# eikehmueller/mlmcpathintegral

Measured on AMD Instinct MI355X. Metric: lattice-site-updates/sec, higher is better.
Workload: dtype f64

## Files before the change

mlmcpathintegral_amd/csrc/schwinger_sweeps.hip:

```cpp
#include <stdio.h>
#include <string.h>
#include <stdlib.h>

#include "lattice_sweep.hpp"
#include "schwinger_perm.hpp"
#include "step_envelope.hpp"
#include "vonmises.hpp"

namespace mlmcpi {

#ifdef MLMCPI_STAMPS
extern "C" int mlmcpi_debug_read_stamps(unsigned long long *h_out, uint32_t n_workgroups) {
  MLMCPI_HIP_TRY(hipDeviceSynchronize());
  MLMCPI_HIP_TRY(hipMemcpyFromSymbol(h_out, HIP_SYMBOL(g_stamps), (size_t)n_workgroups * 16 * sizeof(unsigned long long)));
  return MLMCPI_OK;
}
#endif

template <int NT, int S, bool DIRECT = false, class Setup, class Commit>
__device__ __forceinline__ void heatbath_region(uint32_t nr, uint32_t nc, const RngKey &key, HbPool &pool, Setup setup,
                                                Commit commit) {
  if (DIRECT) {
    heatbath_cells<NT, S>(nr * nc, key, pool,
                          [&](uint32_t idx, double &tau, double &centre, uint32_t &site, uint32_t &o) {
                            const uint32_t ri = idx / nc;
                            setup(ri, idx - ri * nc, tau, centre, site, o);
                          },
                          commit);
    return;
  }
  uint32_t cur = threadIdx.x, ri = cur / nc, ci = cur - ri * nc;
  const uint32_t dr = NT / nc, dc = NT - dr * nc;
  heatbath_cells<NT, S>(nr * nc, key, pool,
                        [&](uint32_t idx, double &tau, double &centre, uint32_t &site, uint32_t &o) {
                          while (cur < idx) {
                            cur += NT;
                            ri += dr;
                            ci += dc;
                            if (ci >= nc) {
                              ci -= nc;
                              ++ri;
                            }
                          }
                          setup(ri, ci, tau, centre, site, o);
                        },
                        commit);
}

template <int NT, int S, bool DIRECT, class E, class Setup, class KappaExact, class Commit>
__device__ __forceinline__ void heatbath_region_step(uint32_t nr, uint32_t nc, uint32_t origin, uint32_t row_stride,
                                                     uint32_t col_stride, const RngKey &key, VsPool<E> &pool, Setup setup,
                                                     KappaExact kappa_exact, Commit commit) {
  if (DIRECT) {
    heatbath_cells_step<NT, S, E>(nr * nc, key, pool,
                                  [&](uint32_t idx) {
                                    const uint32_t ri = idx / nc;
                                    return origin + ri * row_stride + (idx - ri * nc) * col_stride;
                                  },
                                  setup, kappa_exact, commit);
    return;
  }
  const float rcp = 1.0f / (float)nc;
  heatbath_cells_step<NT, S, E>(nr * nc, key, pool,
                                [&](uint32_t idx) {
                                  uint32_t ri = (uint32_t)(((float)idx + 0.5f) * rcp);
                                  int32_t ci = (int32_t)(idx - ri * nc);
                                  if (ci < 0) { --ri; ci += (int32_t)nc; }
                                  else if (ci >= (int32_t)nc) { ++ri; ci -= (int32_t)nc; }
                                  return origin + ri * row_stride + (uint32_t)ci * col_stride;
                                },
                                setup, kappa_exact, commit);
}

template <bool HEAT, int NT, int TWC = 0, int THC = 0, bool STEP = false>
__global__ void __launch_bounds__(NT, HEAT ? (NT == 256 ? 4 : NT == 512 ? 2 : 1) : 1)
    schwinger_sweep_kernel(uint32_t Mt, uint32_t Mx, double beta, const double2 *__restrict__ in,
                           double2 *__restrict__ out, TileGeom tg, uint32_t nsweeps_arg, uint32_t kinds, RngKey key0,
                           uint32_t pool_cap, int qoi_op, double *__restrict__ qoi_partial, const uint32_t *__restrict__ vs_table) {
  extern __shared__ double lds[];
  __shared__ double qoi_red[NT / kWave];
  constexpr bool FIXED = TWC > 0;
  const uint32_t nsweeps = FIXED ? 1u : nsweeps_arg;
  const uint32_t H = 2 * nsweeps;
  const uint32_t tile = blockIdx.x, b = blockIdx.y;
  const uint32_t ty = tile / tg.tiles_x, tx = tile - ty * tg.tiles_x;
  const uint32_t i0 = tx * (FIXED ? TWC : tg.TW), j0 = ty * (FIXED ? THC : tg.TH);
  const uint32_t ow = FIXED ? TWC : min(tg.TW, Mt - i0), oh = FIXED ? THC : min(tg.TH, Mx - j0);
  const uint32_t bw = ow + 2 * H, bh = oh + 2 * H;
  auto wrap = [&](uint32_t base, uint32_t off, uint32_t n) {
    if (FIXED) {
      const uint32_t v = base + off;
      return v >= n ? v - n : v;
    }
    return wrap_add(base, off, n);
  };
  using PoolEntry = typename std::conditional<FIXED, uint16_t, uint32_t>::type;
  double *pool_lds = lds;
  HbPool pool = HbPool::carve(pool_lds, HEAT && !STEP ? pool_cap : 0u);
  VsPool<PoolEntry> vpool = VsPool<PoolEntry>::carve(pool_lds, HEAT && STEP ? pool_cap : 0u, STEP ? vs_table : nullptr);
  double *th0 = lds + (HEAT ? sweep_pool_bytes(STEP, FIXED, pool_cap) / sizeof(double) : 0), *th1 = th0 + (size_t)bw * bh;
  const double beta2 = 2. * beta;
  const uint32_t sc = (uint32_t)(((uint64_t)i0 + Mt - (H % Mt)) % Mt);
  const uint32_t sr = (uint32_t)(((uint64_t)j0 + Mx - (H % Mx)) % Mx);
  const double2 *src = in + (size_t)b * Mt * Mx;
  RngKey key = key0;
  key.chain += b;

  stage_region<NT, (NT >= 1024 ? 3 : 5), double2>(
      bh, bw, [&](uint32_t r, uint32_t c) { return src[(size_t)wrap(sr, r, Mx) * Mt + wrap(sc, c, Mt)]; },
      [&](uint32_t r, uint32_t c, double2 v) {
        th0[r * bw + c] = v.x;
        th1[r * bw + c] = v.y;
      });
  __syncthreads();

  for (uint32_t s = 0; s < nsweeps; ++s) {
    const bool heat = HEAT && (FIXED || ((kinds >> s) & 1u));
    RngKey skey = key;
    skey.step += s;
    const bool last = s + 1 == nsweeps;
    const uint32_t r_hi0 = last ? H + oh : bh - 2;
    const uint32_t c_lo0 = last ? H - 1 : 0, c_hi0 = last ? H + ow : bw - 2;
    const uint32_t r_lo1 = last ? H : 0, r_hi1 = last ? H + oh - 1 : bh - 2;
    for (uint32_t par = 0; par < 2; ++par) {
      const uint32_t r_first = last ? H + par : (par ? 1 : 2);
      const uint32_t nr = r_first <= r_hi0 ? (r_hi0 - r_first) / 2 + 1 : 0;
      const uint32_t ncol = c_hi0 - c_lo0 + 1;
      if (heat && STEP) {
        heatbath_region_step<NT, 5, FIXED, PoolEntry>(
            nr, ncol, r_first * bw + c_lo0, 2 * bw, 1, skey, vpool,
            [&](uint32_t o, VsCell &cell) {
              const uint32_t r = o / bw, c = o - r * bw;
              vs_cell(beta2, th0[o + bw] + th1[o] - th1[o + 1], th0[o - bw] + th1[o - bw + 1] - th1[o - bw], cell);
              cell.site = 2 * (wrap(sr, r, Mx) * Mt + wrap(sc, c, Mt));
            },
            [&](uint32_t o) {
              return vs_kappa_exact(beta2, th0[o + bw] + th1[o] - th1[o + 1], th0[o - bw] + th1[o - bw + 1] - th1[o - bw]);
            },
            [&](uint32_t o, double v) { th0[o] = v; });
      } else if (heat) {
        heatbath_region<NT, 5, FIXED>(
            nr, ncol, skey, pool,
            [&](uint32_t ri, uint32_t ci, double &tau, double &centre, uint32_t &site, uint32_t &o) {
              const uint32_t r = r_first + 2 * ri, c = c_lo0 + ci;
              o = r * bw + c;
              const double tp = th0[o + bw] + th1[o] - th1[o + 1];
              const double tm = th0[o - bw] + th1[o - bw + 1] - th1[o - bw];
              expcos_params(beta, tp, tm, tau, centre);
              site = 2 * (wrap(sr, r, Mx) * Mt + wrap(sc, c, Mt));
            },
            [&](uint32_t o, double v) { th0[o] = v; });
      } else
      for_region<NT>(nr, ncol, [&](uint32_t ri, uint32_t ci) {
        const uint32_t r = r_first + 2 * ri, o = r * bw + c_lo0 + ci;
        const double tp = th0[o + bw] + th1[o] - th1[o + 1];
        const double tm = th0[o - bw] + th1[o - bw + 1] - th1[o - bw];
        th0[o] = mod_2pi_fast((tp + tm) - th0[o]);
      });
      __syncthreads();
    }
    for (uint32_t par = 0; par < 2; ++par) {
      const uint32_t c_first = last ? H + par : (par ? 1 : 2);
      const uint32_t c_hi1 = last ? (par ? H + ow - 1 : H + ow) : bw - 2;
      const uint32_t nc = c_first <= c_hi1 ? (c_hi1 - c_first) / 2 + 1 : 0;
      const uint32_t nrow = r_hi1 - r_lo1 + 1;
      if (heat && STEP) {
        heatbath_region_step<NT, 5, FIXED, PoolEntry>(
            nrow, nc, r_lo1 * bw + c_first, bw, 2, skey, vpool,
            [&](uint32_t o, VsCell &cell) {
              const uint32_t r = o / bw, c = o - r * bw;
              vs_cell(beta2, th0[o] + th1[o + 1] - th0[o + bw], th0[o + bw - 1] + th1[o - 1] - th0[o - 1], cell);
              cell.site = 2 * (wrap(sr, r, Mx) * Mt + wrap(sc, c, Mt)) + 1;
            },
            [&](uint32_t o) {
              return vs_kappa_exact(beta2, th0[o] + th1[o + 1] - th0[o + bw], th0[o + bw - 1] + th1[o - 1] - th0[o - 1]);
            },
            [&](uint32_t o, double v) { th1[o] = v; });
      } else if (heat) {
        heatbath_region<NT, 5, FIXED>(
            nrow, nc, skey, pool,
            [&](uint32_t ri, uint32_t ci, double &tau, double &centre, uint32_t &site, uint32_t &o) {
              const uint32_t r = r_lo1 + ri, c = c_first + 2 * ci;
              o = r * bw + c;
              const double tp = th0[o] + th1[o + 1] - th0[o + bw];
              const double tm = th0[o + bw - 1] + th1[o - 1] - th0[o - 1];
              expcos_params(beta, tp, tm, tau, centre);
              site = 2 * (wrap(sr, r, Mx) * Mt + wrap(sc, c, Mt)) + 1;
            },
            [&](uint32_t o, double v) { th1[o] = v; });
      } else
      for_region<NT>(nrow, nc, [&](uint32_t ri, uint32_t ci) {
        const uint32_t r = r_lo1 + ri, c = c_first + 2 * ci, o = r * bw + c;
        const double tp = th0[o] + th1[o + 1] - th0[o + bw];
        const double tm = th0[o + bw - 1] + th1[o - 1] - th0[o - 1];
        th1[o] = mod_2pi_fast((tp + tm) - th1[o]);
      });
      __syncthreads();
    }
  }

  double acc[1] = {0.0};
  double2 *dst = out + (size_t)b * Mt * Mx;
  for_region<NT>(oh, ow, [&](uint32_t r, uint32_t c) {
    const uint32_t o = (r + H) * bw + (c + H);
    dst[(size_t)(j0 + r) * Mt + (i0 + c)] = make_double2(th0[o], th1[o]);
    if (qoi_op) {
      const double thp = th0[o] + th1[o + 1] - th0[o + bw] - th1[o];
      acc[0] += qoi_op == 3 ? cos_reduced(thp) : mod_2pi(thp);
    }
  });
  if (qoi_op) {
    block_sum<1>(acc, qoi_red);
    if (threadIdx.x == 0) qoi_partial[(size_t)b * gridDim.x + blockIdx.x] = acc[0];
  }
}

template <int NT, bool STEP>
__device__ __forceinline__ void schwinger_image_heat(double *th0, double *th1, VsPool<uint32_t> &vpool, HbPool &hpool, uint32_t Mt,
                                                     uint32_t Mx, double beta, double2 *__restrict__ out, uint32_t i0, uint32_t j0,
                                                     uint32_t b, uint32_t tile, RngKey key0, int qoi_op,
                                                     double *__restrict__ qoi_partial, double *qoi_red) {
  constexpr int TW = 64, TH = 64, HB = 2, IW = TW + 2 * HB;
  constexpr uint32_t bw = IW;
  const uint32_t sc = i0 >= (uint32_t)HB ? i0 - HB : i0 + Mt - HB;
  const uint32_t sr = j0 >= (uint32_t)HB ? j0 - HB : j0 + Mx - HB;
  auto wrap = [](uint32_t base, uint32_t off, uint32_t n) {
    const uint32_t v = base + off;
    return v >= n ? v - n : v;
  };
  RngKey skey = key0;
  skey.chain += b;
  const double beta2 = 2. * beta;
  constexpr bool kMapped = STEP && 32 % (NT / kWave) == 0;
  constexpr uint32_t NW = NT / kWave, NIT = kMapped ? 32 / NW : 1;
  constexpr int kT1 = IW * (TH + 2 * HB) * 8;
  const uint32_t lds_th0 = (uint32_t)(uintptr_t)th0;
  const uint32_t wave = __builtin_amdgcn_readfirstlane(threadIdx.x / kWave), lane = threadIdx.x % kWave;
  for (uint32_t par = 0; par < 2; ++par) {
    const uint32_t r_first = HB + par, nr = (HB + TH - r_first) / 2 + 1;
    constexpr uint32_t ncol = TW + 2;
    if (!STEP)
      heatbath_region<NT, 5, true>(
          nr, ncol, skey, hpool,
          [&](uint32_t ri, uint32_t ci, double &tau, double &centre, uint32_t &site, uint32_t &o) {
            const uint32_t r = r_first + 2 * ri, c = HB - 1 + ci;
            o = r * bw + c;
            expcos_params(beta, th0[o + bw] + th1[o] - th1[o + 1], th0[o - bw] + th1[o - bw + 1] - th1[o - bw], tau, centre);
            site = 2 * (wrap(sr, r, Mx) * Mt + wrap(sc, c, Mt));
          },
          [&](uint32_t o, double v) { th0[o] = v; });
    else if constexpr (kMapped) {
      uint32_t o_next = (r_first + 2 * wave) * bw + (HB - 1) + lane;
      uint32_t srow = wrap(sr, r_first + 2 * wave, Mx);
      const uint32_t scol = wrap(sc, HB - 1 + lane, Mt), n_top = (nr - NIT * NW) * ncol;
      heatbath_cells_step_mapped<NT, NIT, uint32_t>(
          n_top + 2 * (NIT * NW), skey, vpool,
          [&](uint32_t &o, uint32_t &site) {
            o = o_next;
            site = (srow * Mt + scol) << 1;
            o_next += 2 * NW * bw;
            srow = wrap(srow, 2 * NW, Mx);
          },
          [&](uint32_t i) {
            const uint32_t j = i - n_top, ri = i < n_top ? (uint32_t)(NIT * NW) : j >> 1, ci = i < n_top ? i : 64 + (j & 1u);
            return (r_first + 2 * ri) * bw + (HB - 1) + ci;
          },
          [&](uint32_t o) {
            const uint32_t r = o / bw, c = o - r * bw;
            return 2 * (wrap(sr, r, Mx) * Mt + wrap(sc, c, Mt));
          },
          [&](uint32_t o, double (&v)[6]) {
            const uint32_t a = lds_th0 + (o - bw) * 8u;
            v[0] = lds_read_f64<2 * bw * 8>(a);
            v[1] = lds_read_f64<kT1 + bw * 8>(a);
            v[2] = lds_read_f64<kT1 + bw * 8 + 8>(a);
            v[3] = lds_read_f64<0>(a);
            v[4] = lds_read_f64<kT1 + 8>(a);
            v[5] = lds_read_f64<kT1>(a);
          },
          [&](const double (&v)[6], VsCell &cell) { vs_cell(beta2, v[0] + v[1] - v[2], v[3] + v[4] - v[5], cell); },
          [&](uint32_t o) {
            return vs_kappa_exact(beta2, th0[o + bw] + th1[o] - th1[o + 1], th0[o - bw] + th1[o - bw + 1] - th1[o - bw]);
          },
          [&](uint32_t o, double v) { th0[o] = v; });
    } else
    heatbath_region_step<NT, 5, true, uint32_t>(
        nr, ncol, r_first * bw + (HB - 1), 2 * bw, 1, skey, vpool,
        [&](uint32_t o, VsCell &cell) {
          const uint32_t r = o / bw, c = o - r * bw;
          vs_cell(beta2, th0[o + bw] + th1[o] - th1[o + 1], th0[o - bw] + th1[o - bw + 1] - th1[o - bw], cell);
          cell.site = 2 * (wrap(sr, r, Mx) * Mt + wrap(sc, c, Mt));
        },
        [&](uint32_t o) {
          return vs_kappa_exact(beta2, th0[o + bw] + th1[o] - th1[o + 1], th0[o - bw] + th1[o - bw + 1] - th1[o - bw]);
        },
        [&](uint32_t o, double v) { th0[o] = v; });
    __syncthreads();
    MLMCPI_STAMP(5 + par);
  }
  for (uint32_t par = 0; par < 2; ++par) {
    const uint32_t c_first = HB + par, c_hi1 = par ? HB + TW - 1 : HB + TW;
    const uint32_t nc = (c_hi1 - c_first) / 2 + 1;
    if (!STEP)
      heatbath_region<NT, 5, true>(
          TH, nc, skey, hpool,
          [&](uint32_t ri, uint32_t ci, double &tau, double &centre, uint32_t &site, uint32_t &o) {
            const uint32_t r = HB + ri, c = c_first + 2 * ci;
            o = r * bw + c;
            expcos_params(beta, th0[o] + th1[o + 1] - th0[o + bw], th0[o + bw - 1] + th1[o - 1] - th0[o - 1], tau, centre);
            site = 2 * (wrap(sr, r, Mx) * Mt + wrap(sc, c, Mt)) + 1;
          },
          [&](uint32_t o, double v) { th1[o] = v; });
    else if constexpr (kMapped) {
      const uint32_t r0 = HB + 2 * wave + (lane >> 5), c0 = c_first + 2 * (lane & 31u);
      uint32_t o_next = r0 * bw + c0;
      uint32_t rowmt = wrap(sr, r0, Mx) * Mt;
      const uint32_t scol = wrap(sc, c0, Mt), mxmt = Mx * Mt;
      heatbath_cells_step_mapped<NT, NIT, uint32_t>(
          (nc - 32) * (uint32_t)TH, skey, vpool,
          [&](uint32_t &o, uint32_t &site) {
            o = o_next;
            site = ((rowmt + scol) << 1) | 1u;
            o_next += 2 * NW * bw;
            rowmt += 2 * NW * Mt;
            rowmt = min(rowmt, rowmt - mxmt);
          },
          [&](uint32_t i) { return (HB + i) * bw + c_first + 64; },
          [&](uint32_t o) {
            const uint32_t r = o / bw, c = o - r * bw;
            return 2 * (wrap(sr, r, Mx) * Mt + wrap(sc, c, Mt)) + 1;
          },
          [&](uint32_t o, double (&v)[6]) {
            const uint32_t a = lds_th0 + (o - 1) * 8u;
            v[0] = lds_read_f64<8>(a);
            v[1] = lds_read_f64<kT1 + 16>(a);
            v[2] = lds_read_f64<bw * 8 + 8>(a);
            v[3] = lds_read_f64<bw * 8>(a);
            v[4] = lds_read_f64<kT1>(a);
            v[5] = lds_read_f64<0>(a);
          },
          [&](const double (&v)[6], VsCell &cell) { vs_cell(beta2, v[0] + v[1] - v[2], v[3] + v[4] - v[5], cell); },
          [&](uint32_t o) {
            return vs_kappa_exact(beta2, th0[o] + th1[o + 1] - th0[o + bw], th0[o + bw - 1] + th1[o - 1] - th0[o - 1]);
          },
          [&](uint32_t o, double v) { th1[o] = v; });
    } else
    heatbath_region_step<NT, 5, true, uint32_t>(
        TH, nc, HB * bw + c_first, bw, 2, skey, vpool,
        [&](uint32_t o, VsCell &cell) {
          const uint32_t r = o / bw, c = o - r * bw;
          vs_cell(beta2, th0[o] + th1[o + 1] - th0[o + bw], th0[o + bw - 1] + th1[o - 1] - th0[o - 1], cell);
          cell.site = 2 * (wrap(sr, r, Mx) * Mt + wrap(sc, c, Mt)) + 1;
        },
        [&](uint32_t o) {
          return vs_kappa_exact(beta2, th0[o] + th1[o + 1] - th0[o + bw], th0[o + bw - 1] + th1[o - 1] - th0[o - 1]);
        },
        [&](uint32_t o, double v) { th1[o] = v; });
    __syncthreads();
    MLMCPI_STAMP(7 + par);
  }

  double acc[1] = {0.0};
  double2 *dst = out + (size_t)b * Mt * Mx;
  for_region<NT>(TH, TW, [&](uint32_t r, uint32_t c) {
    if (j0 + r >= Mx || i0 + c >= Mt) return;
    const uint32_t o = (r + HB) * bw + (c + HB);
    store_streaming(&dst[(size_t)(j0 + r) * Mt + (i0 + c)], th0[o], th1[o]);
    if (qoi_op) {
      const double thp = th0[o] + th1[o + 1] - th0[o + bw] - th1[o];
      acc[0] += qoi_op == 3 ? cos_reduced(thp) : mod_2pi(thp);
    }
  });
  if (qoi_op) {
    block_sum<1>(acc, qoi_red);
    if (threadIdx.x == 0) qoi_partial[(size_t)b * gridDim.x + tile] = acc[0];
  }
  MLMCPI_STAMP(9);
}

template <int TH>
__global__ void __launch_bounds__(512, 4)
    schwinger_perm_kernel(uint32_t Mt, uint32_t Mx, const double2 *__restrict__ in, double2 *__restrict__ out, uint32_t tiles_x,
                          uint32_t K) {
  constexpr int NT = 512;
  using PG = PermGeom<NT, 0, TH>;
  extern __shared__ double lds[];
  const uint32_t tile = blockIdx.x, b = blockIdx.y;
  const uint32_t ty = tile / tiles_x, tx = tile - ty * tiles_x;
  const uint32_t i0 = tx * 64, j0 = ty * TH;
  double2 res[2][PG::NV];
  perm_sweeps<NT, 0, TH>(lds, in + (size_t)b * Mt * Mx, Mt, Mx, i0, j0, K, res);
  double *th0 = lds, *th1 = lds + 64 * TH;
  __syncthreads();
  perm_store_image<NT, 0, TH>(th0, th1, res);
  __syncthreads();
  double2 *dst = out + (size_t)b * Mt * Mx;
#pragma unroll
  for (int k = 0; k < 64 * TH / NT; ++k) {
    const uint32_t v = threadIdx.x + k * NT, r = v / 64, c = v % 64;
    if (j0 + r < Mx && i0 + c < Mt)
      store_streaming(&dst[(size_t)(j0 + r) * Mt + (i0 + c)], th0[v], th1[v]);
  }
}

template <int NT, bool STEP>
__global__ void __launch_bounds__(NT, 4)
    schwinger_perm_heat_kernel(uint32_t Mt, uint32_t Mx, double beta, const double2 *__restrict__ in, double2 *__restrict__ out,
                               uint32_t tiles_x, uint32_t K, RngKey key0, int qoi_op, double *__restrict__ qoi_partial,
                               const uint32_t *__restrict__ vs_table) {
  using PH = PermHeatGeom<NT, STEP>;
  using PG = typename PH::PG;
  using OH = typename PH::OH;
  constexpr int IW = OH::IW, IH = OH::IH;
  static_assert(PG::OW == IW && 2 * PG::HR == IH, "the closed-form stage fills the heat bath's image");
  extern __shared__ double lds[];
  __shared__ double qoi_red[NT / kWave];
  const uint32_t tile = blockIdx.x, b = blockIdx.y;
  const uint32_t ty = tile / tiles_x, tx = tile - ty * tiles_x;
  const uint32_t i0 = tx * 64, j0 = ty * 64;
  MLMCPI_STAMP(0);
  MLMCPI_STAMP_WHERE();
  uint32_t tabw = 0;
  if (STEP && threadIdx.x < kVsTableBytes / 4) tabw = vs_table[threadIdx.x];
  HbPool hpool = HbPool::carve(lds, STEP ? 0u : OH::hb_pool_cap);
  double *th0 = lds + OH::pool_bytes / sizeof(double), *th1 = th0 + IW * IH;
  double2 res[2][PG::NV];
  perm_sweeps<NT, 2>(th0, in + (size_t)b * Mt * Mx, Mt, Mx, i0, j0, K, res);
  MLMCPI_STAMP(3);
  VsPool<uint32_t> vpool = VsPool<uint32_t>::carve(lds, OH::pool_cap, nullptr);
  if (STEP) {
    if (threadIdx.x < kVsTableBytes / 4) reinterpret_cast<uint32_t *>(lds)[threadIdx.x] = tabw;
    if (threadIdx.x < 2) vpool.count[threadIdx.x] = 0;
    vpool.tab = VsTable::at(lds, vs_table);
  }
  __syncthreads();
  perm_store_image<NT, 2>(th0, th1, res);
  __syncthreads();
  MLMCPI_STAMP(4);
  schwinger_image_heat<NT, STEP>(th0, th1, vpool, hpool, Mt, Mx, beta, out, i0, j0, b, tile, key0, qoi_op, qoi_partial, qoi_red);
}

template <bool HEAT, int NT>
static int allow_full_lds() {
  MLMCPI_HIP_TRY(hipFuncSetAttribute((const void *)schwinger_sweep_kernel<HEAT, NT>, hipFuncAttributeMaxDynamicSharedMemorySize, 160 * 1024 - 256));
  if (HEAT)
    MLMCPI_HIP_TRY(hipFuncSetAttribute((const void *)schwinger_sweep_kernel<HEAT, NT, 0, 0, HEAT>, hipFuncAttributeMaxDynamicSharedMemorySize, 160 * 1024 - 256));
  return MLMCPI_OK;
}

int schwinger_allow_lds() {
  if (int rc = allow_full_lds<false, 256>()) return rc;
  if (int rc = allow_full_lds<true, 256>()) return rc;
  if (int rc = allow_full_lds<false, 512>()) return rc;
  if (int rc = allow_full_lds<true, 512>()) return rc;
  if (int rc = allow_full_lds<false, 1024>()) return rc;
  if (int rc = allow_full_lds<true, 1024>()) return rc;
  if (int rc = schwinger_or_block_allow_lds()) return rc;
  if (int rc = allow_lds((const void *)schwinger_perm_kernel<64>, kPermPlaneMax)) return rc;
  if (int rc = allow_lds((const void *)schwinger_perm_kernel<32>, kPermPlaneMax)) return rc;
  if (int rc = allow_lds((const void *)schwinger_perm_heat_kernel<512, true>, HeatImageGeom::hb_bytes)) return rc;
  if (int rc = allow_lds((const void *)schwinger_perm_heat_kernel<512, false>, HeatImageGeom::hb_bytes)) return rc;
  if (int rc = allow_lds((const void *)schwinger_perm_heat_kernel<1024, true>, 156 * 1024)) return rc;
  if (int rc = allow_lds((const void *)schwinger_perm_heat_kernel<1024, false>, 156 * 1024)) return rc;
  return MLMCPI_OK;
}

template <bool HEAT, int NT>
static void launch_tile_sweep_nt(const SweepLaunch &l, const SweepArgs &a) {
  const dim3 grid(l.grid_x, a.B);
  const TileGeom tg{l.tile_w, l.tile_h, l.tiles_x};
  const uint32_t n = l.n_overrelax + l.n_heatbath;
#define MLMCPI_SCHW_SWEEP(...)                                                                                                       \
  hipLaunchKernelGGL((schwinger_sweep_kernel<__VA_ARGS__>), grid, dim3(NT), l.lds_bytes, a.st, a.Mt, a.Mx, a.coupling, (const double2 *)a.src, \
                     (double2 *)a.dst, tg, n, l.kinds, a.key, l.pool_cap, a.qoi_op, a.qoi_partial, a.vs_table)
  if (l.fixed_tile && l.step) MLMCPI_SCHW_SWEEP(HEAT, NT, 64, 32, HEAT);
  else if (l.fixed_tile) MLMCPI_SCHW_SWEEP(HEAT, NT, 64, 32);
  else if (l.step) MLMCPI_SCHW_SWEEP(HEAT, NT, 0, 0, HEAT);
  else MLMCPI_SCHW_SWEEP(HEAT, NT);
#undef MLMCPI_SCHW_SWEEP
}

static int launch_tile_sweep(const SweepLaunch &l, const SweepArgs &a) {
  const bool heat = l.n_heatbath != 0;
  switch (l.threads) {
    case 1024: heat ? launch_tile_sweep_nt<true, 1024>(l, a) : launch_tile_sweep_nt<false, 1024>(l, a); break;
    case 512: heat ? launch_tile_sweep_nt<true, 512>(l, a) : launch_tile_sweep_nt<false, 512>(l, a); break;
    default: heat ? launch_tile_sweep_nt<true, 256>(l, a) : launch_tile_sweep_nt<false, 256>(l, a);
  }
  MLMCPI_LAUNCH_CHECK("lattice sweep kernel");
  return MLMCPI_OK;
}

static int launch_perm(const SweepLaunch &l, const SweepArgs &a) {
  const dim3 grid(l.grid_x, a.B);
  const double2 *in = (const double2 *)a.src;
  double2 *out = (double2 *)a.dst;
#define MLMCPI_PERM_HEAT(NT, STEP)                                                                                           \
  hipLaunchKernelGGL((schwinger_perm_heat_kernel<NT, STEP>), grid, dim3(NT), l.lds_bytes, a.st, a.Mt, a.Mx, a.coupling, in, out, \
                     l.tiles_x, l.n_overrelax, a.key, a.qoi_op, a.qoi_partial, a.vs_table)
  if (l.kernel == MLMCPI_K_SCHWINGER_PERM_HEAT) {
    if (l.threads == 1024 && l.step) MLMCPI_PERM_HEAT(1024, true);
    else if (l.threads == 1024) MLMCPI_PERM_HEAT(1024, false);
    else if (l.step) MLMCPI_PERM_HEAT(512, true);
    else MLMCPI_PERM_HEAT(512, false);
  } else if (l.tile_h == 64)
    hipLaunchKernelGGL(schwinger_perm_kernel<64>, grid, dim3(512), l.lds_bytes, a.st, a.Mt, a.Mx, in, out, l.tiles_x, l.n_overrelax);
  else
    hipLaunchKernelGGL(schwinger_perm_kernel<32>, grid, dim3(512), l.lds_bytes, a.st, a.Mt, a.Mx, in, out, l.tiles_x, l.n_overrelax);
#undef MLMCPI_PERM_HEAT
  MLMCPI_LAUNCH_CHECK("schwinger closed-form kernel");
  return MLMCPI_OK;
}

int schwinger_sweep_launch(const SweepLaunch &l, const SweepArgs &args) {
  SweepArgs a = args;
  if (l.n_heatbath) a.key.step += l.n_overrelax;
  void *partial = nullptr;
  if (l.step)
    if (int rc = vs_table_device(2. * a.coupling, &a.vs_table)) return rc;
  if (a.qoi_op)
    if (int rc = scratch((size_t)a.B * l.grid_x * sizeof(double), &partial, a.st)) return rc;
  a.qoi_partial = (double *)partial;
  int rc;
  switch (l.kernel) {
    case MLMCPI_K_SCHWINGER_PERM:
    case MLMCPI_K_SCHWINGER_PERM_HEAT: rc = launch_perm(l, a); break;
    case MLMCPI_K_SCHWINGER_OR_BLOCK: rc = schwinger_or_block_launch(l, a); break;
    default: rc = launch_tile_sweep(l, a);
  }
  if (!rc && a.qoi_op) rc = lattice_finish(a.qoi_partial, l.grid_x, a.B, a.qoi_op, 1.0 / ((double)a.Mx * a.Mt), a.d_qoi, a.d_acc, a.st);
  return rc;
}

int schwinger_site_updates(const mlmcpi_lattice_action *act, double *d_state, uint32_t B, const uint32_t *d_sites, uint32_t n,
                           uint32_t site, int32_t heat, uint64_t seed, uint32_t chain0, uint32_t step, hipStream_t st) {
  const uint32_t *vs_table = nullptr;
  if (heat && 2. * act->beta <= kVsKappaMax)
    if (int rc = vs_table_device(2. * act->beta, &vs_table)) return rc;
  hipLaunchKernelGGL((lattice_site_update_kernel<true>), dim3((B + 63) / 64), dim3(64), 0, st, act->Mt, act->Mx, act->beta, d_state, B,
                     d_sites, n, site, (int)heat, make_key(seed, chain0, step), vs_table);
  MLMCPI_LAUNCH_CHECK("lattice_site_update_kernel");
  return MLMCPI_OK;
}

}
```

mlmcpathintegral_amd/csrc/step_envelope.hpp:

```cpp
#pragma once
#include "device_common.hpp"
#include "vonmises.hpp"

namespace mlmcpi {

constexpr double kVsKappaMax = 16.0;
constexpr int kVsClasses = 8, kVsBins = 8, kVsSel = 64;
constexpr uint32_t kVsU2Bits = 22;
constexpr uint32_t kVsCodeOff = 0, kVsScrOff = 512, kVsLwOff = 576, kVsFinOff = 1088, kVsConstOff = 1216, kVsTableBytes = 1232;
__host__ __device__ constexpr uint32_t vs_edge16(uint32_t k) { return (0xC8643210u >> (4u * k)) & 15u; }
__host__ __device__ constexpr uint32_t vs_width16(uint32_t k) { return (0x44221111u >> (4u * k)) & 15u; }
constexpr float kVsU2Slack = 1100.0f;
__host__ __device__ inline float vs_band_of_scale(double scale) { return (float)(1e-5 * (1.0 + scale * 1.4426950408889634)); }

struct VsTable {
  const uint8_t *base;
  float s_acc, s_rej;
  __device__ static VsTable at(const void *image, const uint32_t *__restrict__ d_table) {
    VsTable t{(const uint8_t *)image, 0.f, 0.f};
    if (d_table) {
      t.s_acc = __uint_as_float(to_vgpr(d_table[kVsConstOff / 4]));
      t.s_rej = __uint_as_float(to_vgpr(d_table[kVsConstOff / 4 + 1]));
    }
    return t;
  }
  __device__ static VsTable stage(void *lds, const uint32_t *__restrict__ d_table) {
    if (d_table)
      for (uint32_t i = threadIdx.x; i < kVsTableBytes / 4; i += blockDim.x) ((uint32_t *)lds)[i] = d_table[i];
    return at(lds, d_table);
  }
  __device__ static VsTable in_global(const uint32_t *__restrict__ d_table) { return at(d_table, d_table); }
};

__device__ __forceinline__ float sinf_half_pi(float y) {
  const float y2 = y * y;
  float p = 2.600053086e-06f;
  p = fmaf(p, y2, -1.980661437e-04f);
  p = fmaf(p, y2, 8.333017279e-03f);
  p = fmaf(p, y2, -1.666665710e-01f);
  return fmaf(y * y2, p, y);
}

struct VsCell {
  double centre;
  float kp;
  uint32_t cls;
  uint32_t site;
};

__device__ __forceinline__ void vs_cell(double scale, double x_p, double x_m, VsCell &c) {
  const double v = (x_m - x_p) * (0.25 / kPi);
  const double t = fabs(v - rint(v));
  c.centre = fma(0.5, x_p + x_m, t > 0.25 ? kPi : 0.0);
  const double w = fabs(t - 0.25);
  c.cls = min((uint32_t)(32.0 * w), (uint32_t)(kVsClasses - 1)) * kVsSel;
  c.kp = fmaxf((float)scale * fabsf(sinf_half_pi(fmaf(-6.28318531f, (float)t, 1.57079633f))), 0.0f) * 1.44269504f;
}
__device__ __forceinline__ double vs_kappa_exact(double scale, double x_p, double x_m) {
  return vm_clamp(scale * fabs(cos_half(x_m - x_p)));
}

__device__ __forceinline__ double vs_theta(uint32_t lo, uint32_t hi, uint32_t code, const VsTable &tab) {
  const double m = __hiloint2double((int)(((hi >> 12) & 0x3FFFu) | 0x3FF00000u), (int)__builtin_amdgcn_alignbit(hi, lo << 23, 12));
  const double2 f = *(const double2 *)(tab.base + kVsFinOff + 2u * code);
  return (kPi / 16.0) * fma(f.x, m, f.y);
}

__device__ __forceinline__ float vs_accept_prob(uint32_t hi, float kp, uint32_t cls, const VsTable &tab, uint32_t &code) {
  const uint8_t *row = tab.base + cls;
  code = row[hi >> 26];
  const float2 scr = *(const float2 *)(tab.base + kVsScrOff + code);
  const float sn = sinf_half_pi(fmaf(scr.y, (float)(hi << 6), scr.x));
  return __builtin_amdgcn_exp2f(fmaf(kp, sn - 1.0f, *(const float *)(row + kVsLwOff + code)));
}

__device__ __forceinline__ int vs_exact(uint32_t lo, uint32_t hi, uint32_t code, double tail, double kappa, float lw, const VsTable &tab) {
  const double u2 = ((double)(lo >> (32 - kVsU2Bits)) + tail) * (1.0 / (double)(1u << kVsU2Bits));
  const double la = fma(kappa, cospi_unit(vs_theta(lo, hi, code, tab) * (1.0 / kPi)) - 1.0, 0.69314718055994531 * (double)lw);
  return (u2 <= 0.0 || log_unit(u2) <= la) ? 1 : 0;
}

__device__ __attribute__((noinline)) uint32_t vs_exact_pair(uint32_t k0, uint32_t k1, uint32_t chain, uint32_t step, uint32_t site,
                                                            uint32_t w3, U4 q, uint32_t codes, float lwa, float lwb, double kappa,
                                                            int sa, int sb, const uint8_t *tab_base) {
  const VsTable tab{tab_base, 0.f, 0.f};
  const U4 e = philox4x32_10(site, chain, step, w3 | kVmRefine, k0, k1);
  if (sa < 0) sa = vs_exact(q.x, q.y, codes & 0xFFu, u01(e.x, e.y), kappa, lwa, tab);
  if (sa == 0 && sb < 0) sb = vs_exact(q.z, q.w, codes >> 8, u01(e.z, e.w), kappa, lwb, tab);
  return (uint32_t)(sa & 3) | ((uint32_t)(sb & 3) << 2);
}

template <class KappaExact>
__device__ __forceinline__ bool vs_attempt_pair(const RngKey &k, const PhiloxVKeys *vk, uint32_t site, uint32_t pair, float kp, uint32_t cls,
                                                const VsTable &tab, KappaExact kappa_exact, double &theta, bool &negative,
                                                uint32_t sub0 = 0) {
  const uint32_t w3 = (P_VONMISES << 24) | sub0 | pair;
  const U4 q = vk ? philox4x32_10(site, k.chain, k.step, w3, k.k0, k.k1, *vk) : philox4x32_10(site, k.chain, k.step, w3, k.k0, k.k1);
  uint32_t ca, cb;
  const float pa = vs_accept_prob(q.y, kp, cls, tab, ca), pb = vs_accept_prob(q.w, kp, cls, tab, cb);
  const float la = (float)q.x, lb = (float)q.z;
  bool acc_a = la <= fmaf(pa, tab.s_acc, -kVsU2Slack), acc_b = lb <= fmaf(pb, tab.s_acc, -kVsU2Slack);
  if (!acc_a) {
    const bool rej_a = la >= fmaf(pa, tab.s_rej, kVsU2Slack), rej_b = lb >= fmaf(pb, tab.s_rej, kVsU2Slack);
    if (!rej_a || (!acc_b && !rej_b)) {
      const uint8_t *row = tab.base + cls + kVsLwOff;
      const uint32_t r = vs_exact_pair(k.k0, k.k1, k.chain, k.step, site, w3, q, ca | (cb << 8), *(const float *)(row + ca),
                                       *(const float *)(row + cb), kappa_exact(), rej_a ? 0 : -1, acc_b ? 1 : rej_b ? 0 : -1, tab.base);
      acc_a = (r & 3u) == 1u;
      acc_b = (r >> 2) == 1u;
    }
  }
  const bool first = acc_a;
  const uint32_t lo = first ? q.x : q.z, hi = first ? q.y : q.w;
  theta = vs_theta(lo, hi, first ? ca : cb, tab);
  negative = (lo & 0x200u) != 0;
  return acc_a || acc_b || pair + 1 >= kMaxVmPairs;
}

template <class E>
struct VsPool {
  static constexpr uint32_t kOffBits = sizeof(E) == 2 ? 12 : 16;
  static constexpr uint32_t kMaxPair = (1u << (8 * sizeof(E) - kOffBits)) - 1;
  E *buf;
  uint32_t *count;
  uint32_t cap, use;
  VsTable tab;
  static __host__ __device__ constexpr size_t bytes(uint32_t cap) { return kVsTableBytes + 16 + ((size_t)cap * sizeof(E) + 7) / 8 * 8; }
  __device__ static VsPool carve(double *lds, uint32_t cap, const uint32_t *d_table) {
    VsPool p;
    p.tab = VsTable::stage(lds, d_table);
    p.count = (uint32_t *)((uint8_t *)lds + kVsTableBytes);
    p.buf = (E *)(p.count + 4);
    p.cap = cap;
    p.use = 0;
    if (d_table && threadIdx.x < 2) p.count[threadIdx.x] = 0;
    return p;
  }
};

template <int NT, int S, class E, int LEAN = 0, class OffOf, class Setup, class KappaExact, class Commit>
__device__ __forceinline__ void heatbath_cells_step(uint32_t total, const RngKey &key, VsPool<E> &pool, OffOf off_of, Setup setup,
                                                    KappaExact kappa_exact, Commit commit) {
  using P = VsPool<E>;
  constexpr uint32_t kOffMask = (1u << P::kOffBits) - 1;
  uint32_t *const cnt = pool.count + (pool.use & 1u);
  if (pool.cap && threadIdx.x == 0) pool.count[(pool.use & 1u) ^ 1u] = 0;
  PhiloxVKeys vk_;
  if (!LEAN) vk_ = philox_vkeys(key.k0, key.k1);
  const PhiloxVKeys *const vk = LEAN ? nullptr : &vk_;
  auto cell = [&](uint32_t off, uint32_t pair, auto on_list) {
    VsCell c;
    setup(off, c);
    double th = 0.0;
    bool neg = false;
    for (;;) {
      if (vs_attempt_pair(key, vk, c.site, pair, c.kp, c.cls, pool.tab, [&] { return kappa_exact(off); }, th, neg)) {
        commit(off, mod_2pi_fast(c.centre + (neg ? -th : th)));
        return;
      }
      ++pair;
      if ((bool)on_list && pair == 1 && pool.cap) {
        const uint32_t slot = atomicAdd(cnt, 1u);
        if (slot < pool.cap) {
          pool.buf[slot] = (E)(off | (pair << P::kOffBits));
          return;
        }
      }
    }
  };
  const uint32_t n_main = pool.cap ? total / NT * NT : total;
  if (LEAN >= 2) {
    uint32_t n = n_main, n_list = 0;
    for (int pass = 0; pass < 2; ++pass) {
      for (uint32_t i = threadIdx.x; i < n; i += NT) {
        uint32_t off, pair = 0;
        if (pass == 0) {
          off = off_of(i);
        } else if (i < n_list) {
          const uint32_t e = pool.buf[i];
          off = e & kOffMask;
          pair = e >> P::kOffBits;
        } else {
          off = off_of(n_main + (i - n_list));
        }
        cell(off, pair, pass == 0);
      }
      if (!pool.cap) break;
      if (pass == 0) {
        __syncthreads();
        n_list = min(*cnt, pool.cap);
        n = n_list + (total - n_main);
      }
    }
    ++pool.use;
    return;
  }
  for (uint32_t i = threadIdx.x; i < n_main; i += NT) cell(off_of(i), 0u, std::true_type{});
  if (pool.cap) {
    __syncthreads();
    const uint32_t n_list = min(*cnt, pool.cap);
    const uint32_t n = n_list + (total - n_main);
    for (uint32_t i = threadIdx.x; i < n; i += NT) {
      uint32_t off, pair = 0;
      if (i < n_list) {
        const uint32_t e = pool.buf[i];
        off = e & kOffMask;
        pair = e >> P::kOffBits;
      } else {
        off = off_of(n_main + (i - n_list));
      }
      cell(off, pair, std::false_type{});
    }
  }
  ++pool.use;
}

template <int NT, int NIT, class E, class Main, class Left, class SiteOf, class StencilLoad, class StencilCell, class KappaExact, class Commit>
__device__ __forceinline__ void heatbath_cells_step_mapped(uint32_t n_left, const RngKey &key, VsPool<E> &pool, Main main_cell, Left left_off,
                                                           SiteOf site_of, StencilLoad stencil_load, StencilCell stencil_cell,
                                                           KappaExact kappa_exact, Commit commit) {
  using P = VsPool<E>;
  constexpr uint32_t kOffMask = (1u << P::kOffBits) - 1;
  uint32_t *const cnt = pool.count + (pool.use & 1u);
  if (threadIdx.x == 0) pool.count[(pool.use & 1u) ^ 1u] = 0;
  const PhiloxVKeys vk_ = philox_vkeys(key.k0, key.k1);
  const PhiloxVKeys *const vk = &vk_;
  auto cell = [&](uint32_t off, uint32_t site, uint32_t pair, auto on_list) {
    VsCell c;
    double sv[6];
    stencil_load(off, sv);
    lds_wait6(sv);
    stencil_cell(sv, c);
    double th = 0.0;
    bool neg = false;
    for (;;) {
      if (vs_attempt_pair(key, vk, site, pair, c.kp, c.cls, pool.tab, [&] { return kappa_exact(off); }, th, neg)) {
        commit(off, mod_2pi_fast(c.centre + (neg ? -th : th)));
        return;
      }
      ++pair;
      if ((bool)on_list && pair == 1) {
        const uint32_t slot = atomicAdd(cnt, 1u);
        if (slot < pool.cap) {
          pool.buf[slot] = (E)(off | (pair << P::kOffBits));
          return;
        }
      }
    }
  };
#ifndef MLMCPI_HB_CELLS1
  static_assert(NIT % 2 == 0, "rounds come in pairs");
  for (int k = 0; k < NIT; k += 2) {
    uint32_t off[2], site[2], ca[2], cb[2];
    VsCell c[2];
    U4 q[2];
    float pa[2], pb[2];
    bool acc_a[2], acc_b[2], rej_a[2], rej_b[2];
    double sv[2][6];
#pragma unroll
    for (int j = 0; j < 2; ++j) main_cell(off[j], site[j]);
#pragma unroll
    for (int j = 0; j < 2; ++j) stencil_load(off[j], sv[j]);
    const uint32_t w3 = (P_VONMISES << 24);
#pragma unroll
    for (int j = 0; j < 2; ++j) q[j] = philox4x32_10(site[j], key.chain, key.step, w3, key.k0, key.k1, vk_);
    lds_wait12(sv[0], sv[1]);
#pragma unroll
    for (int j = 0; j < 2; ++j) stencil_cell(sv[j], c[j]);
#pragma unroll
    for (int j = 0; j < 2; ++j) {
      pa[j] = vs_accept_prob(q[j].y, c[j].kp, c[j].cls, pool.tab, ca[j]);
      pb[j] = vs_accept_prob(q[j].w, c[j].kp, c[j].cls, pool.tab, cb[j]);
    }
    bool open = false;
#pragma unroll
    for (int j = 0; j < 2; ++j) {
      const float la = (float)q[j].x, lb = (float)q[j].z;
      acc_a[j] = la <= fmaf(pa[j], pool.tab.s_acc, -kVsU2Slack);
      acc_b[j] = lb <= fmaf(pb[j], pool.tab.s_acc, -kVsU2Slack);
      rej_a[j] = la >= fmaf(pa[j], pool.tab.s_rej, kVsU2Slack);
      rej_b[j] = lb >= fmaf(pb[j], pool.tab.s_rej, kVsU2Slack);
      open = open || (!acc_a[j] && (!rej_a[j] || (!acc_b[j] && !rej_b[j])));
    }
    if (open) {
#pragma unroll
      for (int j = 0; j < 2; ++j)
        if (!acc_a[j] && (!rej_a[j] || (!acc_b[j] && !rej_b[j]))) {
          const uint8_t *row = pool.tab.base + c[j].cls + kVsLwOff;
          const uint32_t r = vs_exact_pair(key.k0, key.k1, key.chain, key.step, site[j], w3, q[j], ca[j] | (cb[j] << 8), *(const float *)(row + ca[j]),
                                           *(const float *)(row + cb[j]), kappa_exact(off[j]), rej_a[j] ? 0 : -1, acc_b[j] ? 1 : rej_b[j] ? 0 : -1,
                                           pool.tab.base);
          acc_a[j] = (r & 3u) == 1u;
          acc_b[j] = (r >> 2) == 1u;
        }
    }
#pragma unroll
    for (int j = 0; j < 2; ++j) {
      if (acc_a[j] || acc_b[j]) {
        const bool first = acc_a[j];
        const uint32_t lo = first ? q[j].x : q[j].z, hi = first ? q[j].y : q[j].w;
        const double th = vs_theta(lo, hi, first ? ca[j] : cb[j], pool.tab);
        commit(off[j], mod_2pi_fast(c[j].centre + ((lo & 0x200u) ? -th : th)));
      } else {
        const uint32_t slot = atomicAdd(cnt, 1u);
        if (slot < pool.cap) pool.buf[slot] = (E)(off[j] | (1u << P::kOffBits));
        else cell(off[j], site[j], 1u, std::false_type{});
      }
    }
  }
#else
  for (int k = 0; k < NIT; ++k) {
    uint32_t off, site;
    main_cell(off, site);
    cell(off, site, 0u, std::true_type{});
  }
#endif
  __syncthreads();
  const uint32_t n_list = min(*cnt, pool.cap);
  const uint32_t n = n_list + n_left;
  for (uint32_t i = threadIdx.x; i < n; i += NT) {
    uint32_t off, pair = 0;
    if (i < n_list) {
      const uint32_t e = pool.buf[i];
      off = e & kOffMask;
      pair = e >> P::kOffBits;
    } else {
      off = left_off(i - n_list);
    }
    cell(off, site_of(off), pair, std::false_type{});
  }
  ++pool.use;
}

__device__ __forceinline__ double vs_draw(const RngKey &k, uint32_t site, double scale, double x_p, double x_m, const VsTable &tab) {
  VsCell c;
  vs_cell(scale, x_p, x_m, c);
  double th = 0.0;
  bool neg = false;
  for (uint32_t pair = 0; !vs_attempt_pair(k, (const PhiloxVKeys *)nullptr, site, pair, c.kp, c.cls, tab, [&] { return vs_kappa_exact(scale, x_p, x_m); }, th, neg); ++pair) {
  }
  return mod_2pi_fast(c.centre + (neg ? -th : th));
}

}
```

Before: 1042 billion.

## Process leftover heatbath cells in a staged round before the spill list

Leftover cells that previously went through the serial tail loop (mixed with spilled list entries) are now handled in an extra staged round with the same batched Philox/stencil/accept pipeline, one cell per lane, with a live mask. Cells that do not fill a whole wave are pushed onto the retry list instead. The per-cell retry helper now issues the first Philox draw before waiting on LDS, overlapping RNG with stencil loads. This aims to cut the divergent serial tail after the barrier, at the cost of more code, a readfirstlane-gated extra round, and timing stamps.

```diff
diff --git a/mlmcpathintegral_amd/csrc/schwinger_sweeps.hip b/mlmcpathintegral_amd/csrc/schwinger_sweeps.hip
--- a/mlmcpathintegral_amd/csrc/schwinger_sweeps.hip
+++ b/mlmcpathintegral_amd/csrc/schwinger_sweeps.hip
@@ -254,16 +254,18 @@
       uint32_t srow = wrap(sr, r_first + 2 * wave, Mx);
       const uint32_t scol = wrap(sc, HB - 1 + lane, Mt), n_top = (nr - NIT * NW) * ncol;
       heatbath_cells_step_mapped<NT, NIT, uint32_t>(
-          n_top + 2 * (NIT * NW), skey, vpool,
+          2 * (NIT * NW) + n_top / kWave * kWave, n_top % kWave, skey, vpool,
           [&](uint32_t &o, uint32_t &site) {
             o = o_next;
             site = (srow * Mt + scol) << 1;
             o_next += 2 * NW * bw;
             srow = wrap(srow, 2 * NW, Mx);
           },
-          [&](uint32_t i) {
-            const uint32_t j = i - n_top, ri = i < n_top ? (uint32_t)(NIT * NW) : j >> 1, ci = i < n_top ? i : 64 + (j & 1u);
-            return (r_first + 2 * ri) * bw + (HB - 1) + ci;
+          [&](uint32_t q, uint32_t &o, uint32_t &site) {
+            const bool top = q >= 2 * (NIT * NW);
+            const uint32_t r = r_first + 2 * (top ? (uint32_t)(NIT * NW) : q >> 1), c = (HB - 1) + (top ? q - 2 * (NIT * NW) : 64 + (q & 1u));
+            o = r * bw + c;
+            site = 2 * (wrap(sr, r, Mx) * Mt + wrap(sc, c, Mt));
           },
           [&](uint32_t o) {
             const uint32_t r = o / bw, c = o - r * bw;
@@ -282,7 +284,7 @@
           [&](uint32_t o) {
             return vs_kappa_exact(beta2, th0[o + bw] + th1[o] - th1[o + 1], th0[o - bw] + th1[o - bw + 1] - th1[o - bw]);
           },
-          [&](uint32_t o, double v) { th0[o] = v; });
+          [&](uint32_t o, double v) { th0[o] = v; }, [&] { MLMCPI_STAMP(11 + par); });
     } else
     heatbath_region_step<NT, 5, true, uint32_t>(
         nr, ncol, r_first * bw + (HB - 1), 2 * bw, 1, skey, vpool,
@@ -317,7 +319,7 @@
       uint32_t rowmt = wrap(sr, r0, Mx) * Mt;
       const uint32_t scol = wrap(sc, c0, Mt), mxmt = Mx * Mt;
       heatbath_cells_step_mapped<NT, NIT, uint32_t>(
-          (nc - 32) * (uint32_t)TH, skey, vpool,
+          (nc - 32) * (uint32_t)TH, 0u, skey, vpool,
           [&](uint32_t &o, uint32_t &site) {
             o = o_next;
             site = ((rowmt + scol) << 1) | 1u;
@@ -325,7 +327,10 @@
             rowmt += 2 * NW * Mt;
             rowmt = min(rowmt, rowmt - mxmt);
           },
-          [&](uint32_t i) { return (HB + i) * bw + c_first + 64; },
+          [&](uint32_t q, uint32_t &o, uint32_t &site) {
+            o = (HB + q) * bw + c_first + 64;
+            site = 2 * (wrap(sr, HB + q, Mx) * Mt + wrap(sc, c_first + 64, Mt)) + 1;
+          },
           [&](uint32_t o) {
             const uint32_t r = o / bw, c = o - r * bw;
             return 2 * (wrap(sr, r, Mx) * Mt + wrap(sc, c, Mt)) + 1;
@@ -343,7 +348,7 @@
           [&](uint32_t o) {
             return vs_kappa_exact(beta2, th0[o] + th1[o + 1] - th0[o + bw], th0[o + bw - 1] + th1[o - 1] - th0[o - 1]);
           },
-          [&](uint32_t o, double v) { th1[o] = v; });
+          [&](uint32_t o, double v) { th1[o] = v; }, [&] { MLMCPI_STAMP(13 + par); });
     } else
     heatbath_region_step<NT, 5, true, uint32_t>(
         TH, nc, HB * bw + c_first, bw, 2, skey, vpool,
diff --git a/mlmcpathintegral_amd/csrc/step_envelope.hpp b/mlmcpathintegral_amd/csrc/step_envelope.hpp
--- a/mlmcpathintegral_amd/csrc/step_envelope.hpp
+++ b/mlmcpathintegral_amd/csrc/step_envelope.hpp
@@ -91,11 +91,8 @@
 }
 
 template <class KappaExact>
-__device__ __forceinline__ bool vs_attempt_pair(const RngKey &k, const PhiloxVKeys *vk, uint32_t site, uint32_t pair, float kp, uint32_t cls,
-                                                const VsTable &tab, KappaExact kappa_exact, double &theta, bool &negative,
-                                                uint32_t sub0 = 0) {
-  const uint32_t w3 = (P_VONMISES << 24) | sub0 | pair;
-  const U4 q = vk ? philox4x32_10(site, k.chain, k.step, w3, k.k0, k.k1, *vk) : philox4x32_10(site, k.chain, k.step, w3, k.k0, k.k1);
+__device__ __forceinline__ bool vs_attempt_pair_words(const RngKey &k, uint32_t site, uint32_t pair, uint32_t w3, const U4 &q, float kp,
+                                                      uint32_t cls, const VsTable &tab, KappaExact kappa_exact, double &theta, bool &negative) {
   uint32_t ca, cb;
   const float pa = vs_accept_prob(q.y, kp, cls, tab, ca), pb = vs_accept_prob(q.w, kp, cls, tab, cb);
   const float la = (float)q.x, lb = (float)q.z;
@@ -115,6 +112,15 @@
   theta = vs_theta(lo, hi, first ? ca : cb, tab);
   negative = (lo & 0x200u) != 0;
   return acc_a || acc_b || pair + 1 >= kMaxVmPairs;
+}
+
+template <class KappaExact>
+__device__ __forceinline__ bool vs_attempt_pair(const RngKey &k, const PhiloxVKeys *vk, uint32_t site, uint32_t pair, float kp, uint32_t cls,
+                                                const VsTable &tab, KappaExact kappa_exact, double &theta, bool &negative,
+                                                uint32_t sub0 = 0) {
+  const uint32_t w3 = (P_VONMISES << 24) | sub0 | pair;
+  const U4 q = vk ? philox4x32_10(site, k.chain, k.step, w3, k.k0, k.k1, *vk) : philox4x32_10(site, k.chain, k.step, w3, k.k0, k.k1);
+  return vs_attempt_pair_words(k, site, pair, w3, q, kp, cls, tab, kappa_exact, theta, negative);
 }
 
 template <class E>
@@ -215,26 +221,36 @@
   ++pool.use;
 }
 
-template <int NT, int NIT, class E, class Main, class Left, class SiteOf, class StencilLoad, class StencilCell, class KappaExact, class Commit>
-__device__ __forceinline__ void heatbath_cells_step_mapped(uint32_t n_left, const RngKey &key, VsPool<E> &pool, Main main_cell, Left left_off,
-                                                           SiteOf site_of, StencilLoad stencil_load, StencilCell stencil_cell,
-                                                           KappaExact kappa_exact, Commit commit) {
+#ifdef MLMCPI_HB_LEFT2
+constexpr int kHbLeftCells = 2;
+#else
+constexpr int kHbLeftCells = 1;
+#endif
+struct VsAllLive {
+  constexpr bool operator[](int) const { return true; }
+};
+template <int NT, int NIT, class E, class Main, class Left, class SiteOf, class StencilLoad, class StencilCell, class KappaExact, class Commit,
+          class AtList>
+__device__ __forceinline__ void heatbath_cells_step_mapped(uint32_t n_round, uint32_t n_push, const RngKey &key, VsPool<E> &pool, Main main_cell,
+                                                           Left left_cell, SiteOf site_of, StencilLoad stencil_load, StencilCell stencil_cell,
+                                                           KappaExact kappa_exact, Commit commit, AtList at_list) {
   using P = VsPool<E>;
   constexpr uint32_t kOffMask = (1u << P::kOffBits) - 1;
   uint32_t *const cnt = pool.count + (pool.use & 1u);
   if (threadIdx.x == 0) pool.count[(pool.use & 1u) ^ 1u] = 0;
   const PhiloxVKeys vk_ = philox_vkeys(key.k0, key.k1);
-  const PhiloxVKeys *const vk = &vk_;
-  auto cell = [&](uint32_t off, uint32_t site, uint32_t pair, auto on_list) {
+  auto cell = [&](uint32_t off, uint32_t site, uint32_t pair, auto on_list) __attribute__((always_inline)) {
     VsCell c;
     double sv[6];
     stencil_load(off, sv);
+    uint32_t w3 = (P_VONMISES << 24) | pair;
+    U4 q = philox4x32_10(site, key.chain, key.step, w3, key.k0, key.k1, vk_);
     lds_wait6(sv);
     stencil_cell(sv, c);
     double th = 0.0;
     bool neg = false;
     for (;;) {
-      if (vs_attempt_pair(key, vk, site, pair, c.kp, c.cls, pool.tab, [&] { return kappa_exact(off); }, th, neg)) {
+      if (vs_attempt_pair_words(key, site, pair, w3, q, c.kp, c.cls, pool.tab, [&] { return kappa_exact(off); }, th, neg)) {
         commit(off, mod_2pi_fast(c.centre + (neg ? -th : th)));
         return;
       }
@@ -246,35 +262,42 @@
           return;
         }
       }
-    }
+      w3 = (P_VONMISES << 24) | pair;
+      q = philox4x32_10(site, key.chain, key.step, w3, key.k0, key.k1, vk_);
+    }
+  };
+  auto push = [&](uint32_t off, uint32_t site, uint32_t pair) __attribute__((always_inline)) {
+    const uint32_t slot = atomicAdd(cnt, 1u);
+    if (slot < pool.cap) pool.buf[slot] = (E)(off | (pair << P::kOffBits));
+    else cell(off, site, pair, std::false_type{});
   };
 #ifndef MLMCPI_HB_CELLS1
-  static_assert(NIT % 2 == 0, "rounds come in pairs");
-  for (int k = 0; k < NIT; k += 2) {
-    uint32_t off[2], site[2], ca[2], cb[2];
-    VsCell c[2];
-    U4 q[2];
-    float pa[2], pb[2];
-    bool acc_a[2], acc_b[2], rej_a[2], rej_b[2];
-    double sv[2][6];
-#pragma unroll
-    for (int j = 0; j < 2; ++j) main_cell(off[j], site[j]);
-#pragma unroll
-    for (int j = 0; j < 2; ++j) stencil_load(off[j], sv[j]);
+  auto staged = [&](const auto &off, const auto &site, const auto &live) __attribute__((always_inline)) {
+    constexpr int NC = (int)(sizeof(off) / sizeof(off[0]));
+    static_assert(NC == 1 || NC == 2, "one or two cells per lane");
+    uint32_t ca[NC], cb[NC];
+    VsCell c[NC];
+    U4 q[NC];
+    float pa[NC], pb[NC];
+    bool acc_a[NC], acc_b[NC], rej_a[NC], rej_b[NC];
+    double sv[NC][6];
+#pragma unroll
+    for (int j = 0; j < NC; ++j) stencil_load(off[j], sv[j]);
     const uint32_t w3 = (P_VONMISES << 24);
 #pragma unroll
-    for (int j = 0; j < 2; ++j) q[j] = philox4x32_10(site[j], key.chain, key.step, w3, key.k0, key.k1, vk_);
-    lds_wait12(sv[0], sv[1]);
-#pragma unroll
-    for (int j = 0; j < 2; ++j) stencil_cell(sv[j], c[j]);
-#pragma unroll
-    for (int j = 0; j < 2; ++j) {
+    for (int j = 0; j < NC; ++j) q[j] = philox4x32_10(site[j], key.chain, key.step, w3, key.k0, key.k1, vk_);
+    if constexpr (NC == 2) lds_wait12(sv[0], sv[1]);
+    else lds_wait6(sv[0]);
+#pragma unroll
+    for (int j = 0; j < NC; ++j) stencil_cell(sv[j], c[j]);
+#pragma unroll
+    for (int j = 0; j < NC; ++j) {
       pa[j] = vs_accept_prob(q[j].y, c[j].kp, c[j].cls, pool.tab, ca[j]);
       pb[j] = vs_accept_prob(q[j].w, c[j].kp, c[j].cls, pool.tab, cb[j]);
     }
     bool open = false;
 #pragma unroll
-    for (int j = 0; j < 2; ++j) {
+    for (int j = 0; j < NC; ++j) {
       const float la = (float)q[j].x, lb = (float)q[j].z;
       acc_a[j] = la <= fmaf(pa[j], pool.tab.s_acc, -kVsU2Slack);
       acc_b[j] = lb <= fmaf(pb[j], pool.tab.s_acc, -kVsU2Slack);
@@ -284,7 +307,7 @@
     }
     if (open) {
 #pragma unroll
-      for (int j = 0; j < 2; ++j)
+      for (int j = 0; j < NC; ++j)
         if (!acc_a[j] && (!rej_a[j] || (!acc_b[j] && !rej_b[j]))) {
           const uint8_t *row = pool.tab.base + c[j].cls + kVsLwOff;
           const uint32_t r = vs_exact_pair(key.k0, key.k1, key.chain, key.step, site[j], w3, q[j], ca[j] | (cb[j] << 8), *(const float *)(row + ca[j]),
@@ -295,18 +318,40 @@
         }
     }
 #pragma unroll
-    for (int j = 0; j < 2; ++j) {
+    for (int j = 0; j < NC; ++j) {
+      if (!live[j]) continue;
       if (acc_a[j] || acc_b[j]) {
         const bool first = acc_a[j];
         const uint32_t lo = first ? q[j].x : q[j].z, hi = first ? q[j].y : q[j].w;
         const double th = vs_theta(lo, hi, first ? ca[j] : cb[j], pool.tab);
         commit(off[j], mod_2pi_fast(c[j].centre + ((lo & 0x200u) ? -th : th)));
       } else {
-        const uint32_t slot = atomicAdd(cnt, 1u);
-        if (slot < pool.cap) pool.buf[slot] = (E)(off[j] | (1u << P::kOffBits));
-        else cell(off[j], site[j], 1u, std::false_type{});
-      }
-    }
+        push(off[j], site[j], 1u);
+      }
+    }
+  };
+  static_assert(NIT % 2 == 0, "rounds come in pairs");
+  for (int k = 0; k < NIT; k += 2) {
+    uint32_t off[2], site[2];
+#pragma unroll
+    for (int j = 0; j < 2; ++j) main_cell(off[j], site[j]);
+    staged(off, site, VsAllLive{});
+  }
+  const uint32_t q0 = threadIdx.x * kHbLeftCells;
+  if ((uint32_t)__builtin_amdgcn_readfirstlane(q0) < n_round) {
+    uint32_t off[kHbLeftCells], site[kHbLeftCells];
+    bool live[kHbLeftCells];
+#pragma unroll
+    for (int j = 0; j < kHbLeftCells; ++j) {
+      live[j] = q0 + j < n_round;
+      left_cell(live[j] ? q0 + j : 0u, off[j], site[j]);
+    }
+    staged(off, site, live);
+  }
+  if (threadIdx.x < n_push) {
+    uint32_t off, site;
+    left_cell(n_round + threadIdx.x, off, site);
+    push(off, site, 0u);
   }
 #else
   for (int k = 0; k < NIT; ++k) {
@@ -314,20 +359,18 @@
     main_cell(off, site);
     cell(off, site, 0u, std::true_type{});
   }
+  for (uint32_t q = threadIdx.x; q < n_round + n_push; q += NT) {
+    uint32_t off, site;
+    left_cell(q, off, site);
+    cell(off, site, 0u, std::true_type{});
+  }
 #endif
   __syncthreads();
+  at_list();
   const uint32_t n_list = min(*cnt, pool.cap);
-  const uint32_t n = n_list + n_left;
-  for (uint32_t i = threadIdx.x; i < n; i += NT) {
-    uint32_t off, pair = 0;
-    if (i < n_list) {
-      const uint32_t e = pool.buf[i];
-      off = e & kOffMask;
-      pair = e >> P::kOffBits;
-    } else {
-      off = left_off(i - n_list);
-    }
-    cell(off, site_of(off), pair, std::false_type{});
+  for (uint32_t i = threadIdx.x; i < n_list; i += NT) {
+    const uint32_t e = pool.buf[i], off = e & kOffMask;
+    cell(off, site_of(off), e >> P::kOffBits, std::false_type{});
   }
   ++pool.use;
 }
```

After: 1038 billion. About the same (-0.4%).
